# lbcb-sci/raven

Hardware: AMD Instinct MI355X
Metric: read Gbase/s through overlap+polish (higher is better)
Workload: dtype u32

## Files before the change

### raven_amd/csrc/engine.h

```cpp
#pragma once

#include <atomic>
#include <memory>
#include <mutex>
#include <string>
#include <vector>

#include "common.h"

namespace rvn {

constexpr int kSketchTile = 1024;
constexpr int kMaxWindow = 256;

inline u64 next_reads_serial() {
  static std::atomic<u64> counter{0};
  return ++counter;
}

struct ReadsDev {
  u32 n = 0;
  u64 total_bases = 0;
  u64 n_words = 0;
  DevBuf packed;
// ... 52 lines not shown
  DevBuf ovl_read_off;
  DevBuf filtered;
  bool has_anchors = false;
  DevBuf anchors;
  DevBuf anchor_off;
  DevBuf anchor_cnt;
};

struct StageTimes {
  enum { kSketch, kSort, kIndex, kFilter, kQuery, kMatch, kSegSort, kIntervals, kChain, kCompact, kMerge, kPile,
         kTruncate, kNum };
  double ms[kNum] = {};
  u64 launches[kNum] = {};
};

struct PileState;
struct PileRegion;
struct ResolveState;

struct EngineOptions {
  long long nw_budget_mb = 0;
  long long nw_group_walk = 0;
  long long nw_stripe_lanes = 0;
  long long index_direct_min_keys = 0;
  long long poa_rows_min_windows = -1;
  long long io_threads = 0;
  long long io_slab_mb = 0;
  long long io_ring = 0;
  long long io_zlib = 0;
  long long arena_mb = 0;
  long long arena_margin_mb = 0;
  long long no_arena = 0;
  long long release_always = 0;
  long long polish_join = 0;
  long long polish_sketch_cache_mb = -1;
};
const char* engine_option_names();
long long* engine_option(EngineOptions& o, const char* name);

struct Engine {
  EngineOptions opt;
  std::recursive_mutex mu;
  u32 k, w, bandwidth, chain, matches, gap;
  int device = 0;
  bool val64 = false;
  hipStream_t stream = nullptr;
// ... 164 lines not shown

struct NwJob;
struct NwWindowRec;
struct NwStats {
  u64 n_aligned = 0, n_retries = 0, n_unaligned = 0, n_batches = 0;
  u64 band_cells = 0, sum_distance = 0, store_bytes = 0;
  double ms = 0;
};
struct NwPathSlots {
  std::vector<std::unique_ptr<DevBuf>> blocks;
  std::vector<u64> slot_end;
};
void nw_breakpoints(Engine& e, const ReadsDev& T, const ReadsDev& R, std::vector<NwJob>& jobs, u32 w, NwWindowRec* d_recs,
                    u64 n_recs, NwStats& st, std::vector<u32>* distances = nullptr, NwPathSlots* path = nullptr);
struct NwPaths {
  u32 n = 0, n_not_aligned = 0;
  u64 n_runs = 0, n_ops = 0;
  std::vector<u32> distances;
  DevBuf run_off, runs, op_off;
  double device_ms = 0;
};
void nw_align_paths(Engine& e, const ReadsDev& T, const ReadsDev& Q, std::vector<NwJob>& jobs, NwPaths& out);
void nw_paths_expand(Engine& e, const NwPaths& p, u8* d_ops);
int nw_breakpoints_host(const u64* t_words, u32 t_len, const u64* r_words, u32 r_len, u32 t_begin, u32 n, u32 q_begin, u32 m,
                        int rc, u32 w, u32 k, int force_R, NwWindowRec* recs, u32* distance, u32* band);
void shard_split_minimizers(Engine& e, const u64* d_val, const u64* d_org, u64 n, u32 world, u64* d_val_out, u64* d_org_out,
                            u64* counts );
void shard_split_overlaps(Engine& e, const Overlap* d_ovl, u64 n, const u32* bounds , u32 world, u32 self,
                          Overlap* d_out, u64* counts );
u64 shard_count_flagged(Engine& e, const u64* d_org, u64 n);
void shard_adjacent_diff(Engine& e, const u64* d_seg, u64 n, u64* d_cnt);
void shard_regroup(Engine& e, u32 world, const u64* const* d_cnt, const u64* const* d_grp, const u64* const* d_pos,
                   const u64* n_src , u32 n_reads, u64* d_seg, u64* d_grp_out, u64* d_pos_out);
void shard_lhs_offsets(Engine& e, const Overlap* d_ovl, u64 n, u32 n_reads, u32* d_off);
struct PolishDirectOut {
  u8* out;
  const u64* off;
  u64* len;
};
void polish_map_best(Engine& e, ReadsDev& T, ReadsDev& R, u32 r_first, u32 r_last, double err_thr,
                     std::vector<Overlap>& best, std::vector<u32>& best_t, u64* n_overlaps);
void polish_round(Engine& e, ReadsDev& T, ReadsDev& R, const u8* h_quals, const u64* h_qual_off, double q_thr,
                  double err_thr, u32 w, bool trim, int m, int n, int g, std::vector<std::vector<u8>>& polished,
                  std::vector<double>& ratio, PolishStats& stats, u64 win_first = 0, u64 win_last = ~0ULL,
                  std::vector<u32>* win_count = nullptr, std::vector<u32>* win_polished = nullptr,
                  const PolishDirectOut* direct = nullptr);

struct Pass2State {
// ... 128 lines not shown
```

### raven_amd/csrc/engine.hip

```cpp
#include <chrono>
#include <memory>

#include "abi.h"
#include "poa.h"

using namespace rvn;

static_assert(sizeof(rvn_overlap) == sizeof(rvn::Overlap), "overlap layout");

namespace {

thread_local std::string g_err;

const char* kStageNames[StageTimes::kNum] = {"sketch", "sort", "index", "filter", "query_sketch", "match",
                                             "seg_sort", "intervals", "chain", "compact", "merge", "pile",
                                             "truncate"};

void swap_bufs(DevBuf& a, DevBuf& b) {
  std::swap(a.ptr, b.ptr);
  std::swap(a.cap, b.cap);
}

}

// ... 54 lines not shown
  }
  for (u32 i = first; i < last; ++i) e.c_index_bases += r.h_len[i];
  e.c_index_min += e.index_sketch.count;
  index_build(e, e.index_sketch, !(e.index.has_query_flags || e.index.all_query));
  e.c_index_keys += e.index.u;
  if (raw_handed_over) {
    if (e.raw_sketch.val.cap < e.index_sketch.val.cap) swap_bufs(e.raw_sketch.val, e.index_sketch.val);
    if (e.raw_sketch.org.cap < e.index_sketch.org.cap) swap_bufs(e.raw_sketch.org, e.index_sketch.org);
  }
}

void fetch_values(Engine& e, const DevBuf& val, u64 n, u64* values) {
  if (!values || n == 0) return;
  if (e.val64) {
    RVN_HIP(hipMemcpy(values, val.ptr, n * 8, hipMemcpyDeviceToHost));
  } else {
    std::vector<u32> tmp(n);
    RVN_HIP(hipMemcpy(tmp.data(), val.ptr, n * 4, hipMemcpyDeviceToHost));
    for (u64 i = 0; i < n; ++i) values[i] = tmp[i];
  }
}

const char* engine_option_names() {
  return "nw_budget_mb, nw_group_walk, nw_stripe_lanes, index_direct_min_keys, poa_rows_min_windows, io_threads, io_slab_mb, io_ring, io_zlib, arena_mb, arena_margin_mb, "
         "no_arena, release_always, polish_join, polish_sketch_cache_mb";
}
long long* engine_option(EngineOptions& o, const char* name) {
  const std::string n(name ? name : "");
  if (n == "nw_budget_mb") return &o.nw_budget_mb;
  if (n == "nw_group_walk") return &o.nw_group_walk;
  if (n == "nw_stripe_lanes") return &o.nw_stripe_lanes;
  if (n == "index_direct_min_keys") return &o.index_direct_min_keys;
  if (n == "poa_rows_min_windows") return &o.poa_rows_min_windows;
  if (n == "io_threads") return &o.io_threads;
  if (n == "io_slab_mb") return &o.io_slab_mb;
  if (n == "io_ring") return &o.io_ring;
  if (n == "io_zlib") return &o.io_zlib;
  if (n == "arena_mb") return &o.arena_mb;
  if (n == "arena_margin_mb") return &o.arena_margin_mb;
  if (n == "no_arena") return &o.no_arena;
  if (n == "release_always") return &o.release_always;
  if (n == "polish_join") return &o.polish_join;
  if (n == "polish_sketch_cache_mb") return &o.polish_sketch_cache_mb;
  return nullptr;
}

void engine_release_scratch(Engine& e) {
  if (e.stream) (void)rvn_stream_sync(e.stream);
  e.query_ready = false;
  DevBuf* bufs[] = {
      &e.index.s_val[0], &e.index.s_val[1], &e.index.s_org[0], &e.index.s_org[1], &e.index.u_val, &e.index.u_start,
      &e.index.table, &e.index.direct, &e.index_sketch.val, &e.index_sketch.org, &e.index_sketch.read_off, &e.query_sketch.val,
      &e.query_sketch.org, &e.query_sketch.read_off, &e.raw_sketch.val, &e.raw_sketch.org, &e.raw_sketch.read_off,
      &e.map_out.ovl, &e.map_out.ovl_read_off, &e.map_out.filtered, &e.map_out.anchors, &e.map_out.anchor_off,
// ... 223 lines not shown
```

### raven_amd/csrc/nwpath.hip

```cpp
#include <algorithm>
#include <mutex>
#include <chrono>
#include <cmath>
#include <cstdio>
#include <cstdlib>
#include <exception>
#include <type_traits>
#include <vector>

#include "engine.h"
#include "nwpath.h"
#include "nwsweep.h"
#include "nwtrace.h"
#include "wave.h"

namespace rvn {

namespace {

constexpr int kNwLaneStripCols = 16;
constexpr int kNwGroupLanes = 16;
constexpr u32 kNwGroupWalkMaxJobs = 8192;
constexpr u32 kSideSweepMaxWaves = 2048;
constexpr u32 kLevels = 8;
// ... 113 lines not shown
        }
        if ((t & 31) == 0) {
          const int qi = (t >> 5) - 1;
          if (st_ok && qi < n_q) {
            NwPm* p = ck_j + static_cast<u64>(qi - qc0) * row + static_cast<u64>(lig) * R;
#pragma unroll
            for (int r = 0; r < R; ++r) p[r] = NwPm{ln.Pv[r], ln.Mv[r]};
          }
        }
        ln.next_group(t);
        if (STRIPED && is_top) top.next_group(t);
      }
    }
    if (STRIPED && has && lig == lig_hand) hs_j[row * static_cast<u64>(gps)] = static_cast<u32>(sc_hand);
    const u32 res1 = group_max<G>(ln.result);
    if (has && lig == 0 && last) {
      const u32 res = res1 - 1u;
      result[ji] = res;
      status[ji] = (res1 != 0 && res <= k) ? 0u : 2u;
    }
  }
}

template <bool STRIP_LDS, int SC, class Out = NwWindowRec>
__global__ __launch_bounds__(64) void nw_trace_kernel(const NwJob* __restrict__ jobs, const u32* __restrict__ idx, u32 n_idx,
                                                      const u64* __restrict__ t_words, const u64* __restrict__ r_words,
                                                      const u32* __restrict__ hs, const NwPm* __restrict__ ck,
                                                      const u32* __restrict__ result, u32* __restrict__ status, u32 w,
                                                      Out* __restrict__ recs, u64* __restrict__ scratch) {
  __shared__ u64 s_pv[STRIP_LDS ? (SC + 1) * 64 : 1];
  __shared__ u64 s_mv[STRIP_LDS ? (SC + 1) * 64 : 1];
  __builtin_amdgcn_s_setprio(3);
  const u32 q = blockIdx.x * 64 + threadIdx.x;
  if (q >= n_idx) return;
  const u32 ji = idx[q];
  if (status[ji] != 0) return;
  const NwJob J = jobs[ji];
  const NwGeo geo = nw_geo_job(J);
  u64* g_pv = scratch + static_cast<u64>(blockIdx.x) * (2 * kNwStripCols * 64);
  const NwStripMem<64> mem{STRIP_LDS ? s_pv : g_pv, STRIP_LDS ? s_mv : g_pv + kNwStripCols * 64, static_cast<int>(threadIdx.x)};
  if constexpr (std::is_same<Out, u32>::value) {
    NwRunSink sink;
    sink.init(recs + J.bp_off, nw_slot_words(J.k));
    status[ji] = static_cast<u32>(nw_trace_job<64, SC, NwRunSink>(J, geo, t_words, r_words, hs + J.hs, ck + J.ckpt, mem, result[ji], w,
                                                                  nullptr, sink));
  } else {
// ... 36 lines not shown
    bad = G.walk_batch(geo, t == 0);
    __threadfence_block();
    __builtin_amdgcn_wave_barrier();
    if (bad) break;
  }
  const int rcode = bad ? 1 : G.wk.finish(t == 0);
  if (t == 0) status[ji] = static_cast<u32>(rcode);
}

template <int R, int G, bool STRIPED = false>
void launch_sweep(Engine& e, hipStream_t s, const NwJob* d_jobs, const u32* d_idx, u32 n_idx, const ReadsDev& T, const ReadsDev& Rd,
                  u32* d_hs, NwPm* d_ck, u32* d_result, u32* d_status, u32* d_next, int stripe = 0) {
  if (n_idx == 0) return;
  constexpr u32 NG = 64 / G;
  const u32 bundles = (n_idx + NG - 1) / NG;
  const u32 per_simd = static_cast<u32>(sweep_waves_per_simd<R>());
  const u32 waves = std::min<u32>(bundles, 256u * 4u * (per_simd > 4 ? per_simd - 2 : per_simd));
  RVN_HIP(hipMemsetAsync(d_next, 0, 4, s));
  RVN_KLAUNCH_ON(kKNwForward, s, (nw_sweep_kernel<R, G, STRIPED><<<(waves + 3) / 4, 256, 0, s>>>(
                               d_jobs, d_idx, n_idx, T.packed.as<u64>(), Rd.packed.as<u64>(), d_hs, d_ck, d_result,
                               d_status, d_next, stripe)));
}

u32 kcap_of(u32 n, u32 m, u32 R, u32 G) {
  const u32 d = n > m ? n - m : m - n;
  const u64 room = static_cast<u64>(G) * (64ULL * R + 1) - 64ULL * R;
  if (room < d) return 0;
  const u64 k = d + ((room - d) / 2) * 2 + 1;
  return static_cast<u32>(std::min<u64>(k, static_cast<u64>(n) + m));
}

u32 level_of(const NwJob& J) {
  if (J.S) return kStriped;
  for (u32 x = 0; x < kLevels; ++x)
    if (kRs[x] == J.R && kGs[x] == J.G) return x;
  return kLevels - 1;
}

}

void nw_breakpoints(Engine& e, const ReadsDev& T, const ReadsDev& Rd, std::vector<NwJob>& jobs, u32 w,
                    NwWindowRec* d_recs, u64 n_recs, NwStats& st, std::vector<u32>* distances, NwPathSlots* path) {
  st = NwStats();
  const u32 nj = static_cast<u32>(jobs.size());
  if (distances) distances->assign(nj, ~0u);
  if (path) path->slot_end.assign(nj, 0);
  hipStream_t s = e.stream;
  if (n_recs) RVN_HIP(hipMemsetAsync(d_recs, 0xFF, n_recs * sizeof(NwWindowRec), s));
  if (nj == 0) return;
  RVN_HIP(hipEventRecord(e.ev0, s));
  if (!e.nw_streams[0]) {
    int prio_least = 0, prio_greatest = 0;
    RVN_HIP(hipDeviceGetStreamPriorityRange(&prio_least, &prio_greatest));
    constexpr int kNwEv = static_cast<int>(sizeof(e.nw_ev) / sizeof(e.nw_ev[0]));
    hipStream_t made[8] = {nullptr, nullptr, nullptr, nullptr, nullptr, nullptr, nullptr, nullptr};
    hipEvent_t made_ev[kNwEv + 4] = {};
    try {
      for (int b = 0; b < 8; ++b) {
        if (b >= 3 && prio_greatest != prio_least)
          RVN_HIP(hipStreamCreateWithPriority(&made[b], hipStreamNonBlocking, prio_greatest));
        else
// ... 8 lines not shown
      throw;
    }
    for (int b = 0; b < 3; ++b) e.nw_side[b] = made[5 + b];
    for (int i = 0; i < 4; ++i) e.nw_side_ev[i] = made_ev[kNwEv + i];
    for (int i = 0; i < kNwEv; ++i) e.nw_ev[i] = made_ev[i];
    for (int b = 0; b < 5; ++b) e.nw_streams[b] = made[b];
  }
  struct WalkGuard {
    Engine& e;
    ~WalkGuard() {
      if (!std::uncaught_exceptions()) return;
      for (hipStream_t st2 : e.nw_streams)
        if (st2) (void)hipStreamSynchronize(st2);
      for (hipStream_t st2 : e.nw_side)
        if (st2) (void)hipStreamSynchronize(st2);
      (void)hipStreamSynchronize(e.stream);
    }
  } walk_guard{e};
  double rate = e.nw_rate > 0 ? e.nw_rate : 0.13;
  if (const char* ev = knob("RVN_NW_RATE")) rate = std::atof(ev);
  u64 budget = 0;
  const u32 stripe_lanes = e.opt.nw_stripe_lanes > 0 && e.opt.nw_stripe_lanes < 64 ? static_cast<u32>(e.opt.nw_stripe_lanes) : 64u;

  auto plan = [&](NwJob& J, u64 k) -> bool {
    const u32 d = J.n > J.m ? J.n - J.m : J.m - J.n;
    k = std::max<u64>(std::max<u64>(k, d), 16);
    k = std::min<u64>(k, static_cast<u64>(J.n) + J.m);
    J.S = 0;
    for (u32 lvl = 0; lvl < kLevels; ++lvl) {
      if (kGs[lvl] > stripe_lanes) continue;
      const u32 cap = kcap_of(J.n, J.m, kRs[lvl], kGs[lvl]);
      if (cap >= k) {
        J.R = kRs[lvl];
        J.G = kGs[lvl];
        J.k = static_cast<u32>(k);
        J.kcap = cap;
        return true;
      }
    }
    const u32 cap = kcap_of(J.n, J.m, 8, kNwMaxStripes * stripe_lanes);
    if (cap < k) return false;
    const NwGeo g = nw_geo_striped(J.n, J.m, static_cast<u32>(k), 8, stripe_lanes);
    if (g.hs_words() * 4 + g.ck_entries() * 16 > budget) return false;
    J.R = 8;
    J.G = 64;
    J.S = stripe_lanes;
    J.k = static_cast<u32>(k);
    J.kcap = cap;
    return true;
  };
  std::vector<u32> valid;
  for (u32 i = 0; i < nj; ++i) {
    const NwJob& J = jobs[i];
    if (J.n == 0 || J.m == 0 || J.n >= (1u << 30) || J.m >= (1u << 30)) ++st.n_unaligned;
    else valid.push_back(i);
  }

  {
    size_t free_b = 0, total_b = 0;
    RVN_HIP(hipMemGetInfo(&free_b, &total_b));
    const u64 held = e.nw_hs.cap + e.nw_ck.cap + e.nw_hs2.cap + e.nw_ck2.cap + e.nw_hs3.cap + e.nw_ck3.cap + e.nw_hs4.cap + e.nw_ck4.cap;
    budget = std::min<u64>((static_cast<u64>(free_b) + devpool::free_total()) / 4 + held, 64ULL << 30);
    if (e.opt.nw_budget_mb > 0) budget = static_cast<u64>(e.opt.nw_budget_mb) << 20;
    budget = std::max<u64>(budget, 64ULL << 20);
  }
  const bool trace_lds = !(knob("RVN_NW_TRACE_MEM") && std::atoi(knob("RVN_NW_TRACE_MEM")) == 1);
  const int group_walk = static_cast<int>(e.opt.nw_group_walk);
  const bool one_stream = knob("RVN_NW_ONE_STREAM") != nullptr;
  const bool dbg_sync = knob("RVN_NW_DEBUG") && std::atoi(knob("RVN_NW_DEBUG")) >= 2;
  std::vector<double> rates;
  rates.reserve(nj);
  std::vector<u32> h_result(nj), h_status(nj);
  constexpr u32 kHeadMax = 4096;
  NwJob* d_jobs = e.nw_jobs.get<NwJob>(static_cast<size_t>(nj) + 1 + 2 * kHeadMax);
  u32* d_res = e.nw_res.get<u32>(3 * static_cast<size_t>(nj) + 32 + 6 * kHeadMax);
  u32* d_status = d_res + nj + 1;
  u32* d_idx = d_status + nj + 1;
  u32* d_next = d_idx + nj + 1;
  struct PassDev {
    NwJob* jobs;
    u32 *idx, *res, *status;
    bool compact;
  };
  const PassDev dev_all{d_jobs, d_idx, d_res, d_status, false};
  const PassDev dev_head{d_jobs + nj + 1, d_next + 4 + 2 * kHeadMax, d_next + 4, d_next + 4 + kHeadMax, true};
  const PassDev dev_retry{dev_head.jobs + kHeadMax, dev_head.idx + 3 * kHeadMax, dev_head.res + 3 * kHeadMax,
                          dev_head.status + 3 * kHeadMax, true};
  u32* d_side_next = d_next + 4 + 6 * kHeadMax;
  bool side_pending[3] = {false, false, false};
  auto join_side = [&]() {
    for (int x = 0; x < 3; ++x) {
      if (side_pending[x]) RVN_HIP(hipStreamWaitEvent(s, e.nw_side_ev[x], 0));
      side_pending[x] = false;
    }
  };
  struct Obs {
    double len, d;
  };
  using clk = std::chrono::steady_clock;
  double h_plan = 0, h_order = 0, h_up = 0, h_res = 0;
  auto since = [](clk::time_point t) { return std::chrono::duration<double, std::milli>(clk::now() - t).count(); };
  std::vector<Obs> obs;
  struct Chunk {
    size_t c0, c1;
    u64 hs_w, ck_e;
    u32 coff[kClasses + 1];
  };
  DevBuf* hs_buf[4] = {&e.nw_hs, &e.nw_hs2, &e.nw_hs3, &e.nw_hs4};
  DevBuf* ck_buf[4] = {&e.nw_ck, &e.nw_ck2, &e.nw_ck3, &e.nw_ck4};
  bool set_used[4] = {false, false, false, false};
  struct Queued {
    std::vector<u32> order;
    PassDev dev;
    bool sweep_only;
    std::vector<u32> res, status;
  };
  std::vector<Queued> queued;
  std::vector<u8> early;
  enum Layout { kOwnFirst, kHeadOnly, kRotating };
  auto enqueue = [&](const std::vector<u32>& todo, bool sweep_only, Layout layout, const PassDev& dev, hipStream_t up,
                     std::vector<u32>* left) {
    if (todo.empty()) return;
    auto t_h = clk::now();
    std::vector<u32> order;
    {
      const size_t nt = todo.size();
      std::vector<u32> key(nt), tmp(nt), idx(nt);
      parallel_for(nt, 16384, [&](size_t x0, size_t x1) {
        for (size_t x = x0; x < x1; ++x) {
          const NwJob& J = jobs[todo[x]];
          const u32 mm = J.S ? std::min<u32>(nw_geo_job(J).n_stripes, (1u << 20) - 1) : std::min<u32>(J.m >> 3, (1u << 20) - 1);
          static_assert(kClasses <= 16, "4 bits of variant + 20 bits of length = the 24 key bits of the two passes");
          key[x] = 0xFFFFFFu - ((level_of(J) << 20) | mm);
          idx[x] = static_cast<u32>(x);
        }
      });
      for (int pass = 0; pass < 2; ++pass) {
        u32 cnt[4097] = {};
        const int sh = 12 * pass;
        for (size_t x = 0; x < nt; ++x) cnt[((key[idx[x]] >> sh) & 4095u) + 1]++;
        for (int c = 0; c < 4096; ++c) cnt[c + 1] += cnt[c];
        for (size_t x = 0; x < nt; ++x) tmp[cnt[(key[idx[x]] >> sh) & 4095u]++] = idx[x];
        idx.swap(tmp);
      }
      order.resize(nt);
      for (size_t x = 0; x < nt; ++x) order[x] = todo[idx[x]];
    }
    std::vector<Chunk> chunks;
    u64 slot_w = 0;
    struct Need {
      u64 hw, ce, cells;
      u32 level;
    };
    std::vector<Need> need(order.size());
    parallel_for(order.size(), 16384, [&](size_t x0, size_t x1) {
      for (size_t x = x0; x < x1; ++x) {
        const NwJob& J = jobs[order[x]];
        const NwGeo g = nw_geo_job(J);
        need[x] = Need{g.hs_words(), g.ck_entries(), static_cast<u64>(J.m) * (static_cast<u64>(g.lo) + g.hi + 1), level_of(J)};
      }
    });
    for (size_t c0 = 0; c0 < order.size();) {
      Chunk C{};
      C.c0 = c0;
      size_t c1 = c0;
      while (c1 < order.size()) {
        NwJob& J = jobs[order[c1]];
        const u64 hw = need[c1].hw, ce = need[c1].ce;
        const u64 share = (chunks.empty() && layout != kRotating) ? budget / 12 : budget / 3;
        if (c1 > c0 && (C.hs_w + hw) * 4 + (C.ck_e + ce) * 16 > share) break;
        J.hs = C.hs_w;
        J.ckpt = C.ck_e;
        if (path && !sweep_only) {
          J.bp_off = slot_w;
          slot_w += nw_slot_words(J.k);
        }
        C.hs_w += hw;
        C.ck_e += ce;
        st.band_cells += need[c1].cells;
        C.coff[need[c1].level + 1]++;
        ++c1;
      }
      u32 run_off = 0, cnt[kClasses];
      for (u32 x = 0; x < kClasses; ++x) cnt[x] = C.coff[x + 1];
      for (int x = static_cast<int>(kClasses) - 1; x >= 0; --x) {
        C.coff[x] = run_off;
        run_off += cnt[x];
      }
      C.coff[kClasses] = run_off;
      C.c1 = c1;
      st.store_bytes = std::max<u64>(st.store_bytes, C.hs_w * 4 + C.ck_e * 16);
      chunks.push_back(C);
      c0 = c1;
      if (layout == kHeadOnly) break;
    }
    if (layout == kHeadOnly && chunks[0].c1 < order.size()) {
      for (size_t x = chunks[0].c1; x < order.size(); ++x) left->push_back(order[x]);
      order.resize(chunks[0].c1);
    }
    auto set_of = [&](size_t ci) -> int {
      if (layout == kRotating) return static_cast<int>(ci % 3);
      return ci == 0 ? 3 : static_cast<int>((ci - 1) % 3);
    };
    for (int b = 0; b < 4; ++b) {
      u64 set_hs = 0, set_ck = 0;
// ... 11 lines not shown
    u64* d_strip = nullptr;
    if (!trace_lds) {
      size_t mc = 0;
      for (const Chunk& C : chunks) mc = std::max(mc, C.c1 - C.c0);
      d_strip = e.nw_strip.get<u64>(static_cast<size_t>((mc + 63) / 64) * 2 * kNwStripCols * 64 * 4 + 64);
    }
    u32* d_slots = nullptr;
    if (path && !sweep_only) {
      path->blocks.emplace_back(new DevBuf());
      d_slots = path->blocks.back()->get<u32>(slot_w + 16);
      for (u32 i : order) path->slot_end[i] = reinterpret_cast<u64>(d_slots + jobs[i].bp_off + nw_slot_words(jobs[i].k) - 1);
    }
    h_order += since(t_h);
    t_h = clk::now();
    if (dev.compact) {
      std::vector<NwJob> hj(order.size());
      std::vector<u32> iota(order.size());
      for (size_t x = 0; x < order.size(); ++x) {
        hj[x] = jobs[order[x]];
        iota[x] = static_cast<u32>(x);
      }
      RVN_HIP(hipMemcpyAsync(dev.jobs, hj.data(), hj.size() * sizeof(NwJob), hipMemcpyHostToDevice, up));
      RVN_HIP(hipMemcpyAsync(dev.idx, iota.data(), iota.size() * 4, hipMemcpyHostToDevice, up));
      RVN_HIP(rvn_stream_sync(up));
    } else {
      RVN_HIP(hipMemcpyAsync(dev.jobs, jobs.data(), static_cast<size_t>(nj) * sizeof(NwJob), hipMemcpyHostToDevice, up));
      RVN_HIP(hipMemcpyAsync(dev.idx, order.data(), order.size() * 4, hipMemcpyHostToDevice, up));
      RVN_HIP(rvn_stream_sync(up));
    }
    h_up += since(t_h);
    for (size_t ci = 0; ci < chunks.size(); ++ci) {
      const Chunk& C = chunks[ci];
      const int b = set_of(ci);
      u32* hs = hs_buf[b]->as<u32>();
      NwPm* ck = ck_buf[b]->as<NwPm>();
      const u32* idx_c = dev.idx + C.c0;
      const u32 cn = static_cast<u32>(C.c1 - C.c0);
      if (set_used[b]) RVN_HIP(hipStreamWaitEvent(s, e.nw_ev[b], 0));
      auto count_of = [&](u32 x) -> u32 {
        const u32 next_off = x == 0 ? cn : C.coff[x - 1];
        return next_off - C.coff[x];
      };
      hipStream_t ts = one_stream ? s : e.nw_streams[b];
      auto launch_walk_to = [&](auto* d_out, hipStream_t wst, const u32* idx_w, u32 n_w) {
        using Out = typename std::remove_pointer<decltype(d_out)>::type;
        if (group_walk == 2 || (group_walk != 1 && n_w <= kNwGroupWalkMaxJobs)) {
          constexpr u32 NG = 64 / kNwGroupLanes;
          RVN_KLAUNCH_ON(kKNwTraceback, wst, (nw_trace_group_kernel<kNwGroupLanes, Out><<<(n_w + NG - 1) / NG, 64, 0, wst>>>(
                                                 dev.jobs, idx_w, n_w, T.packed.as<u64>(), Rd.packed.as<u64>(), hs, ck, dev.res,
                                                 dev.status, w, d_out)));
// ... 3 lines not shown
                                                 dev.status, w, d_out, nullptr)));
        } else if (trace_lds) {
          RVN_KLAUNCH_ON(kKNwTraceback, wst, (nw_trace_kernel<true, kNwCkSteps, Out><<<(n_w + 63) / 64, 64, 0, wst>>>(
                                                 dev.jobs, idx_w, n_w, T.packed.as<u64>(), Rd.packed.as<u64>(), hs, ck, dev.res,
                                                 dev.status, w, d_out, nullptr)));
        } else {
          RVN_KLAUNCH_ON(kKNwTraceback, wst, (nw_trace_kernel<false, kNwCkSteps, Out><<<(n_w + 63) / 64, 64, 0, wst>>>(
                                                 dev.jobs, idx_w, n_w, T.packed.as<u64>(), Rd.packed.as<u64>(), hs, ck, dev.res,
                                                 dev.status, w, d_out,
                                                 d_strip + static_cast<size_t>(b) * ((e.nw_strip.cap / 32) & ~size_t(63)))));
        }
      };
      auto launch_walk = [&](hipStream_t wst, const u32* idx_w, u32 n_w) {
        if (path) launch_walk_to(d_slots, wst, idx_w, n_w);
        else launch_walk_to(d_recs, wst, idx_w, n_w);
      };
      bool side[kLevels] = {};
      bool side_used[3] = {false, false, false};
      {
        u32 n_levels = 0;
        for (u32 x = 0; x < kLevels; ++x) n_levels += count_of(x) ? 1u : 0u;
        if (n_levels >= 2 && !one_stream && !dbg_sync)
          for (u32 x = 0; x < kLevels; ++x) {
            const u32 bundles = (count_of(x) + 64 / kGs[x] - 1) / (64 / kGs[x]);
            side[x] = count_of(x) && bundles <= kSideSweepMaxWaves;
            if (side[x]) side_used[x % 3] = true;
          }
        if (side_used[0] || side_used[1] || side_used[2]) {
          RVN_HIP(hipEventRecord(e.nw_side_ev[3], s));
          for (int y = 0; y < 3; ++y)
            if (side_used[y]) RVN_HIP(hipStreamWaitEvent(e.nw_side[y], e.nw_side_ev[3], 0));
        }
      }
      if (const u32 n_str = count_of(kStriped)) {
        const u32* idx_s = idx_c + C.coff[kStriped];
        std::vector<u32> n_stripes(n_str);
        for (u32 x = 0; x < n_str; ++x) n_stripes[x] = static_cast<u32>(nw_geo_job(jobs[order[C.c0 + C.coff[kStriped] + x]]).n_stripes);
        for (u32 stp = 0;; ++stp) {
          u32 n_st = 0;
          while (n_st < n_str && n_stripes[n_st] > stp) ++n_st;
          if (n_st == 0) break;
          launch_sweep<8, 64, true>(e, s, dev.jobs, idx_s, n_st, T, Rd, hs, ck, dev.res, dev.status, d_next, static_cast<int>(stp));
          if (dbg_sync) {
            RVN_HIP(hipStreamSynchronize(s));
            std::fprintf(stderr, "[raven_hip] nw: stripe %u done, %u jobs\n", stp, n_st);
          }
        }
      }
#define RVN_SWEEP(x, R_, G_)                                                                                         \
  do {                                                                                                               \
    launch_sweep<R_, G_>(e, side[x] ? e.nw_side[(x) % 3] : s, dev.jobs, idx_c + C.coff[x], count_of(x), T, Rd, hs, ck, \
                         dev.res, dev.status, side[x] ? d_side_next + (x) : d_next);                                   \
    if (dbg_sync && count_of(x)) {                                                                                   \
      RVN_HIP(hipStreamSynchronize(s));                                                                              \
      std::fprintf(stderr, "[raven_hip] nw: sweep R=%d G=%d done, %u jobs\n", R_, G_, count_of(x));                   \
    }                                                                                                                \
  } while (0)
      RVN_SWEEP(7, 8, 64);
      RVN_SWEEP(6, 4, 64);
      RVN_SWEEP(5, 2, 64);
      RVN_SWEEP(4, 1, 64);
      RVN_SWEEP(3, 1, 32);
      RVN_SWEEP(2, 1, 16);
      RVN_SWEEP(1, 1, 8);
      RVN_SWEEP(0, 1, 4);
#undef RVN_SWEEP
      for (int y = 0; y < 3; ++y)
        if (side_used[y]) {
          RVN_HIP(hipEventRecord(e.nw_side_ev[y], e.nw_side[y]));
          side_pending[y] = true;
        }
      ++st.n_batches;
      if (sweep_only) continue;
      if (!one_stream) {
        RVN_HIP(hipEventRecord(e.nw_ev[4], s));
        RVN_HIP(hipStreamWaitEvent(ts, e.nw_ev[4], 0));
        for (int y = 0; y < 3; ++y)
          if (side_used[y]) RVN_HIP(hipStreamWaitEvent(ts, e.nw_side_ev[y], 0));
      }
      launch_walk(ts, idx_c, cn);
      if (!one_stream) {
        RVN_HIP(hipEventRecord(e.nw_ev[b], ts));
        set_used[b] = true;
      }
// ... 602 lines not shown
      continue;
    }
    J.R = kRs[lvl];
    J.G = kGs[lvl];
    J.k = static_cast<u32>(kk);
    J.kcap = cap;
    int rcode;
    switch (J.R) {
      case 1: rcode = emulate_job<1>(J, J.G, t_words, r_words, w, recs, distance, band, walk_gl); break;
      case 2: rcode = emulate_job<2>(J, J.G, t_words, r_words, w, recs, distance, band, walk_gl); break;
      case 4: rcode = emulate_job<4>(J, J.G, t_words, r_words, w, recs, distance, band, walk_gl); break;
      default: rcode = emulate_job<8>(J, J.G, t_words, r_words, w, recs, distance, band, walk_gl); break;
    }
    if (walk_gl && band) band[3] = static_cast<u32>(g_group_batches_store);
    if (rcode == -3 && !force_R) {
      kk = std::min<u64>(static_cast<u64>(cap) + 1, static_cast<u64>(n) + m);
      continue;
    }
    return rcode;
  }
  return -3;
}

#endif

}
```

### raven_amd/hip.py

```python
from __future__ import annotations

import ctypes as C
import os

import numpy as np

_HERE = os.path.dirname(os.path.abspath(__file__))
LIB_PATH = os.environ.get("RVN_LIB_PATH") or os.path.join(_HERE, "lib", "libraven_hip.so")
TEST_LIB_PATH = os.path.join(os.path.dirname(LIB_PATH), "libraven_hip_test.so")

OVERLAP_DTYPE = np.dtype([
    ("lhs_id", "<u4"), ("lhs_begin", "<u4"), ("lhs_end", "<u4"),
    ("rhs_id", "<u4"), ("rhs_begin", "<u4"), ("rhs_end", "<u4"),
    ("score", "<u4"), ("strand", "<u4")])

ED_PAIR_DTYPE = np.dtype([
    ("lhs_read", "<u4"), ("lhs_begin", "<u4"), ("lhs_len", "<u4"),
    ("rhs_read", "<u4"), ("rhs_begin", "<u4"), ("rhs_len", "<u4"),
    ("strand", "<u4"), ("reserved", "<u4")])

ALIGN_PAIR_DTYPE = np.dtype([
    ("query_read", "<u4"), ("query_begin", "<u4"), ("query_len", "<u4"),
    ("target_read", "<u4"), ("target_begin", "<u4"), ("target_len", "<u4"),
    ("strand", "<u4"), ("reserved", "<u4")])
# ... 1253 lines not shown


NW_REC_DTYPE = np.dtype([("first_t", "<u4"), ("first_q", "<u4"), ("last_t", "<u4"), ("last_q", "<u4"),
                         ("grid", "<u2", (8,))])


def test_nw_breakpoints(t_words, t_len, r_words, r_len, t_begin, n, q_begin, m, rc, w, k=64, force_r=0, group_lanes=0,
                       stripe_lanes=0, device=False):
    t_words = np.ascontiguousarray(t_words, dtype=np.uint64)
    r_words = np.ascontiguousarray(r_words, dtype=np.uint64)
    n_win = (t_begin + n - 1) // w - t_begin // w + 1
    recs = np.zeros(n_win, dtype=NW_REC_DTYPE)
    dist = np.zeros(1, dtype=np.uint32)
    band = np.zeros(5 if (stripe_lanes or device) else (4 if group_lanes else 3), dtype=np.uint32)
    flags = (1 if rc else 0) | (int(stripe_lanes) << 16) | (1 << 24 if device else int(group_lanes) << 8)
    rc_ = test_lib().rvn_test_nw_breakpoints(_p(t_words), t_len, _p(r_words), r_len, t_begin, n, q_begin, m, flags, w, k,
                                             force_r, _p(recs), _p(dist), _p(band))
    if rc_ < 0:
        raise ValueError("rvn_test_nw_breakpoints: %d" % rc_)
    if device:
        return recs, int(dist[0]), dict(k=int(band[0]), stripe_lanes=int(band[1]), R=int(band[2]), stripes=int(band[3]),
                                        stage_ms=band[4] / 1000.0), rc_
    return recs, int(dist[0]), tuple(int(x) for x in band), rc_
```

Measured before the change: 1.443.

## Pack multiple ring-1 NW sweep jobs into shared 64-lane waves

Adds a packed sweep kernel for R=1 Myers/NW jobs. Each job gets only as many lanes as its band needs, and a host-side bin-packer fills 64-lane wavefronts with several jobs, sorted by step count. Before, a narrow-band job occupied a whole wave. The path is on by default (only disabled when nw_sweep_pack==2) and adds host packing cost, a persistent atomic work queue, and more complex chunking. Idle lanes and mismatched step counts within a wave can still waste work.

```diff
diff --git a/raven_amd/csrc/engine.h b/raven_amd/csrc/engine.h
--- a/raven_amd/csrc/engine.h
+++ b/raven_amd/csrc/engine.h
@@ -98,6 +98,7 @@
   long long nw_budget_mb = 0;
   long long nw_group_walk = 0;
   long long nw_stripe_lanes = 0;
+  long long nw_sweep_pack = 0;
   long long index_direct_min_keys = 0;
   long long poa_rows_min_windows = -1;
   long long io_threads = 0;
@@ -308,8 +309,15 @@
 };
 void nw_align_paths(Engine& e, const ReadsDev& T, const ReadsDev& Q, std::vector<NwJob>& jobs, NwPaths& out);
 void nw_paths_expand(Engine& e, const NwPaths& p, u8* d_ops);
+struct NwPackPlan {
+  std::vector<u32> order, wrec;
+  u32 n_waves() const { return static_cast<u32>(wrec.size() / 3); }
+};
+void nw_pack_waves(const u32* lanes, const u32* steps, u32 n, NwPackPlan& plan);
 int nw_breakpoints_host(const u64* t_words, u32 t_len, const u64* r_words, u32 r_len, u32 t_begin, u32 n, u32 q_begin, u32 m,
                         int rc, u32 w, u32 k, int force_R, NwWindowRec* recs, u32* distance, u32* band);
+int nw_packed_wave_host(const u64* t_words, const u64* r_words, u32 r_len, u32 n_jobs, const u32* spans, u64 ring_starts, u32 w,
+                        NwWindowRec* recs, u32* distance, u32* status, u32* lanes);
 void shard_split_minimizers(Engine& e, const u64* d_val, const u64* d_org, u64 n, u32 world, u64* d_val_out, u64* d_org_out,
                             u64* counts );
 void shard_split_overlaps(Engine& e, const Overlap* d_ovl, u64 n, const u32* bounds , u32 world, u32 self,
diff --git a/raven_amd/csrc/engine.hip b/raven_amd/csrc/engine.hip
--- a/raven_amd/csrc/engine.hip
+++ b/raven_amd/csrc/engine.hip
@@ -100,7 +100,7 @@
 }
 
 const char* engine_option_names() {
-  return "nw_budget_mb, nw_group_walk, nw_stripe_lanes, index_direct_min_keys, poa_rows_min_windows, io_threads, io_slab_mb, io_ring, io_zlib, arena_mb, arena_margin_mb, "
+  return "nw_budget_mb, nw_group_walk, nw_stripe_lanes, nw_sweep_pack, index_direct_min_keys, poa_rows_min_windows, io_threads, io_slab_mb, io_ring, io_zlib, arena_mb, arena_margin_mb, "
          "no_arena, release_always, polish_join, polish_sketch_cache_mb";
 }
 long long* engine_option(EngineOptions& o, const char* name) {
@@ -108,6 +108,7 @@
   if (n == "nw_budget_mb") return &o.nw_budget_mb;
   if (n == "nw_group_walk") return &o.nw_group_walk;
   if (n == "nw_stripe_lanes") return &o.nw_stripe_lanes;
+  if (n == "nw_sweep_pack") return &o.nw_sweep_pack;
   if (n == "index_direct_min_keys") return &o.index_direct_min_keys;
   if (n == "poa_rows_min_windows") return &o.poa_rows_min_windows;
   if (n == "io_threads") return &o.io_threads;
diff --git a/raven_amd/csrc/nwpath.hip b/raven_amd/csrc/nwpath.hip
--- a/raven_amd/csrc/nwpath.hip
+++ b/raven_amd/csrc/nwpath.hip
@@ -159,6 +159,100 @@
   }
 }
 
+__host__ __device__ __forceinline__ void nw_packed_place(u64 starts, int lane, int& ring, int& gbase) {
+  const u64 upto = starts << (63 - lane);
+  ring = static_cast<int>(RVN_POPC64(upto)) - 1;
+#if defined(__HIP_DEVICE_COMPILE__)
+  gbase = lane - __clzll(static_cast<long long>(upto));
+#else
+  gbase = upto ? lane - __builtin_clzll(upto) : -1;
+#endif
+}
+
+__global__ __launch_bounds__(256) __attribute__((amdgpu_waves_per_eu(8)))
+void nw_sweep_packed_kernel(const NwJob* __restrict__ jobs, const u32* __restrict__ idx, const u32* __restrict__ wrec,
+                            u32 n_waves, const u64* __restrict__ t_words, const u64* __restrict__ r_words,
+                            u32* __restrict__ hs, NwPm* __restrict__ ck, u32* __restrict__ result, u32* __restrict__ status,
+                            u32* __restrict__ next) {
+  __shared__ u64 s_peq[4][4 * 64];
+  const int lane = lane_id();
+  u64* peq = s_peq[threadIdx.x >> 6];
+  for (;;) {
+    int lane_f = lane;
+    asm volatile("" : "+v"(lane_f));
+    u32 q0 = atomicAdd(next, lane_f == 0 ? 1u : 0u);
+    q0 = static_cast<u32>(__builtin_amdgcn_readfirstlane(static_cast<int>(q0)));
+    if (q0 >= n_waves) break;
+    u32 starts_lo = wrec[3 * static_cast<u64>(q0)], starts_hi = wrec[3 * static_cast<u64>(q0) + 1];
+    const u32 off = wrec[3 * static_cast<u64>(q0) + 2];
+    NwSweepLane<1, 64> ln;
+    const NwJob* J0 = jobs + idx[off];
+    u32* const hs0 = hs + J0->hs;
+    NwPm* const ck0 = ck + J0->ckpt;
+    u32 hs_o = 0, ck_o = 0;
+    int prev = lane;
+    {
+      int ring, gbase;
+      nw_packed_place(static_cast<u64>(starts_lo) | (static_cast<u64>(starts_hi) << 32), lane_f, ring, gbase);
+      const int lig = lane - gbase;
+      bool has = false;
+      if (ring >= 0) {
+        const NwJob J = jobs[idx[off + static_cast<u32>(ring)]];
+        const NwGeo geo = nw_geo(J.n, J.m, J.k, 1);
+        has = lig < geo.L;
+        if (has) {
+          ln.init(J, t_words, r_words, geo, lig, peq, lane);
+          hs_o = static_cast<u32>(J.hs - J0->hs) + static_cast<u32>(lig);
+          ck_o = static_cast<u32>(J.ckpt - J0->ckpt) + static_cast<u32>(lig);
+          prev = lig == 0 ? gbase + geo.L - 1 : lane - 1;
+        }
+      }
+      if (!has) ln.init_idle(peq, lane);
+    }
+    int n_steps_w = ln.g.m + ln.g.n_super;
+#pragma unroll
+    for (int o = 32; o > 0; o >>= 1) {
+      const int v = __shfl_xor(n_steps_w, o, 64);
+      n_steps_w = v > n_steps_w ? v : n_steps_w;
+    }
+    n_steps_w = __builtin_amdgcn_readfirstlane((n_steps_w + 15) & ~15);
+    __builtin_assume(n_steps_w >= 16);
+    for (int t = 1; t <= n_steps_w; ++t) {
+      const int x = __shfl(ln.xf, prev, 64);
+      if (__ballot(ln.has_event(t)) != 0) {
+        const int sp = __shfl(ln.sc, prev, 64);
+        if (ln.has_event(t)) ln.event(t, x, sp);
+      }
+      ln.step(t, x);
+      if ((t & 15) == 0) {
+        int n_steps = ln.g.m;
+        asm volatile("" : "+v"(n_steps));
+        n_steps += ln.g.n_super;
+        if (t < n_steps + kNwHsSteps) hs0[hs_o] = ln.acc[0];
+        hs_o += static_cast<u32>(ln.g.L);
+        if ((t & 31) == 0) {
+          if (t <= n_steps) ck0[ck_o] = NwPm{ln.Pv[0], ln.Mv[0]};
+          ck_o += static_cast<u32>(ln.g.L);
+        }
+        ln.next_group(t);
+      }
+    }
+    asm volatile("" : "+s"(starts_lo), "+s"(starts_hi));
+    asm volatile("" : "+v"(lane_f));
+    int ring, gbase;
+    nw_packed_place(static_cast<u64>(starts_lo) | (static_cast<u64>(starts_hi) << 32), lane_f, ring, gbase);
+    const int L = ln.g.L;
+    const u64 found = __ballot(ln.result != 0) & ((L >= 64 ? ~0ULL : (1ULL << L) - 1ULL) << (gbase & 63));
+    const u32 res1 = __shfl(ln.result, found ? static_cast<int>(__ffsll(static_cast<unsigned long long>(found))) - 1 : lane, 64);
+    if (ring >= 0 && lane == gbase && L > 0) {
+      const u32 ji = idx[off + static_cast<u32>(ring)];
+      const u32 res = (found ? res1 : 0u) - 1u;
+      result[ji] = res;
+      status[ji] = (found != 0 && res <= jobs[ji].k) ? 0u : 2u;
+    }
+  }
+}
+
 template <bool STRIP_LDS, int SC, class Out = NwWindowRec>
 __global__ __launch_bounds__(64) void nw_trace_kernel(const NwJob* __restrict__ jobs, const u32* __restrict__ idx, u32 n_idx,
                                                       const u64* __restrict__ t_words, const u64* __restrict__ r_words,
@@ -241,6 +335,16 @@
                                d_status, d_next, stripe)));
 }
 
+void launch_sweep_packed(Engine& e, hipStream_t s, const NwJob* d_jobs, const u32* d_idx, const u32* d_wrec, u32 n_waves,
+                         const ReadsDev& T, const ReadsDev& Rd, u32* d_hs, NwPm* d_ck, u32* d_result, u32* d_status, u32* d_next) {
+  if (n_waves == 0) return;
+  const u32 waves = std::min<u32>(n_waves, 256u * 4u * 6u);
+  RVN_HIP(hipMemsetAsync(d_next, 0, 4, s));
+  RVN_KLAUNCH_ON(kKNwForward, s, (nw_sweep_packed_kernel<<<(waves + 3) / 4, 256, 0, s>>>(
+                               d_jobs, d_idx, d_wrec, n_waves, T.packed.as<u64>(), Rd.packed.as<u64>(), d_hs, d_ck, d_result,
+                               d_status, d_next)));
+}
+
 u32 kcap_of(u32 n, u32 m, u32 R, u32 G) {
   const u32 d = n > m ? n - m : m - n;
   const u64 room = static_cast<u64>(G) * (64ULL * R + 1) - 64ULL * R;
@@ -249,13 +353,89 @@
   return static_cast<u32>(std::min<u64>(k, static_cast<u64>(n) + m));
 }
 
-u32 level_of(const NwJob& J) {
+constexpr u32 kPackedLevel = 4;
+u32 level_of(const NwJob& J, bool pack) {
   if (J.S) return kStriped;
+  if (pack && J.R == 1) return kPackedLevel;
   for (u32 x = 0; x < kLevels; ++x)
     if (kRs[x] == J.R && kGs[x] == J.G) return x;
   return kLevels - 1;
 }
 
+}
+
+void nw_pack_waves(const u32* lanes, const u32* steps, u32 n, NwPackPlan& plan) {
+  plan.order.clear();
+  plan.wrec.clear();
+  if (n == 0) return;
+  u32 max_steps = 0;
+  for (u32 i = 0; i < n; ++i) {
+    if (lanes[i] < 1 || lanes[i] > 64) throw HipError("[raven_hip] nw_pack_waves: a ring of 1 .. 64 lanes");
+    max_steps = std::max(max_steps, steps[i]);
+  }
+  std::vector<u64> srt(n), tmp(n);
+  for (u32 i = 0; i < n; ++i) srt[i] = (static_cast<u64>(max_steps - steps[i]) << 32) | i;
+  std::vector<u32> cnt(65537);
+  for (int sh = 0; sh < 32 && (max_steps >> sh) != 0; sh += 16) {
+    std::fill(cnt.begin(), cnt.end(), 0u);
+    for (u32 x = 0; x < n; ++x) cnt[((srt[x] >> (32 + sh)) & 65535u) + 1]++;
+    for (int c = 0; c < 65536; ++c) cnt[c + 1] += cnt[c];
+    for (u32 x = 0; x < n; ++x) tmp[cnt[(srt[x] >> (32 + sh)) & 65535u]++] = srt[x];
+    srt.swap(tmp);
+  }
+  u32 head[66] = {}, end[66] = {};
+  for (u32 i = 0; i < n; ++i) end[lanes[i]]++;
+  for (u32 l = 1, at = 0; l <= 64; ++l) {
+    head[l] = at;
+    at += end[l];
+    end[l] = at;
+  }
+  std::vector<u64>& bkt = tmp;
+  {
+    u32 fill[66];
+    for (u32 l = 0; l < 66; ++l) fill[l] = head[l];
+    for (u32 x = 0; x < n; ++x) {
+      const u32 job = static_cast<u32>(srt[x]);
+      bkt[fill[lanes[job]]++] = (static_cast<u64>(x) << 32) | job;
+    }
+  }
+  u32 top[65];
+  for (u32 l = 0; l <= 64; ++l) top[l] = l >= 1 && head[l] < end[l] ? static_cast<u32>(bkt[head[l]] >> 32) : n;
+  u32 min_l = 1;
+  plan.order.reserve(n);
+  plan.wrec.reserve(3 * static_cast<size_t>(n / 2 + 1));
+  std::vector<u8> placed(static_cast<size_t>(n) + 1, 0);
+  u32 lead = 0;
+  while (plan.order.size() < n) {
+    u32 free_l = 64;
+    u64 starts = 0;
+    const u32 off = static_cast<u32>(plan.order.size());
+    while (placed[lead]) ++lead;
+    while (min_l <= 64 && top[min_l] == n) ++min_l;
+    while (free_l >= min_l) {
+      u32 best = n, bl = 0;
+      if (free_l == 64) {
+        best = lead;
+        bl = lanes[static_cast<u32>(srt[lead])];
+      } else {
+        for (u32 l = min_l; l <= free_l; ++l) {
+          const bool lt = top[l] < best;
+          best = lt ? top[l] : best;
+          bl = lt ? l : bl;
+        }
+        if (best == n) break;
+      }
+      placed[best] = 1;
+      starts |= 1ULL << (64 - free_l);
+      plan.order.push_back(static_cast<u32>(bkt[head[bl]]));
+      ++head[bl];
+      top[bl] = head[bl] < end[bl] ? static_cast<u32>(bkt[head[bl]] >> 32) : n;
+      free_l -= bl;
+    }
+    plan.wrec.push_back(static_cast<u32>(starts));
+    plan.wrec.push_back(static_cast<u32>(starts >> 32));
+    plan.wrec.push_back(off);
+  }
 }
 
 void nw_breakpoints(Engine& e, const ReadsDev& T, const ReadsDev& Rd, std::vector<NwJob>& jobs, u32 w,
@@ -310,6 +490,8 @@
   u64 budget = 0;
   const u32 stripe_lanes = e.opt.nw_stripe_lanes > 0 && e.opt.nw_stripe_lanes < 64 ? static_cast<u32>(e.opt.nw_stripe_lanes) : 64u;
 
+  const bool pack = e.opt.nw_sweep_pack != 2;
+
   auto plan = [&](NwJob& J, u64 k) -> bool {
     const u32 d = J.n > J.m ? J.n - J.m : J.m - J.n;
     k = std::max<u64>(std::max<u64>(k, d), 16);
@@ -317,12 +499,17 @@
     J.S = 0;
     for (u32 lvl = 0; lvl < kLevels; ++lvl) {
       if (kGs[lvl] > stripe_lanes) continue;
+      if (pack && kRs[lvl] == 1 && static_cast<u64>(J.m) + (J.n + 63) / 64 > (1u << 30) - 16) continue;
       const u32 cap = kcap_of(J.n, J.m, kRs[lvl], kGs[lvl]);
       if (cap >= k) {
         J.R = kRs[lvl];
         J.G = kGs[lvl];
         J.k = static_cast<u32>(k);
         J.kcap = cap;
+        if (pack && J.R == 1) {
+          J.G = nw_ring_lanes(nw_band_lo(J.n, J.m, J.k), nw_band_hi(J.n, J.m, J.k), 1);
+          J.kcap = kcap_of(J.n, J.m, 1, J.G);
+        }
         return true;
       }
     }
@@ -361,7 +548,7 @@
   std::vector<u32> h_result(nj), h_status(nj);
   constexpr u32 kHeadMax = 4096;
   NwJob* d_jobs = e.nw_jobs.get<NwJob>(static_cast<size_t>(nj) + 1 + 2 * kHeadMax);
-  u32* d_res = e.nw_res.get<u32>(3 * static_cast<size_t>(nj) + 32 + 6 * kHeadMax);
+  u32* d_res = e.nw_res.get<u32>(6 * static_cast<size_t>(nj) + 40 + 12 * kHeadMax);
   u32* d_status = d_res + nj + 1;
   u32* d_idx = d_status + nj + 1;
   u32* d_next = d_idx + nj + 1;
@@ -369,12 +556,15 @@
     NwJob* jobs;
     u32 *idx, *res, *status;
     bool compact;
+    u32* wrec;
   };
-  const PassDev dev_all{d_jobs, d_idx, d_res, d_status, false};
-  const PassDev dev_head{d_jobs + nj + 1, d_next + 4 + 2 * kHeadMax, d_next + 4, d_next + 4 + kHeadMax, true};
+  u32* d_side_next = d_next + 4 + 6 * kHeadMax;
+  u32* d_wrec = d_side_next + 8;
+  const PassDev dev_all{d_jobs, d_idx, d_res, d_status, false, d_wrec};
+  const PassDev dev_head{d_jobs + nj + 1, d_next + 4 + 2 * kHeadMax, d_next + 4, d_next + 4 + kHeadMax, true,
+                         d_wrec + 3 * (static_cast<size_t>(nj) + 1)};
   const PassDev dev_retry{dev_head.jobs + kHeadMax, dev_head.idx + 3 * kHeadMax, dev_head.res + 3 * kHeadMax,
-                          dev_head.status + 3 * kHeadMax, true};
-  u32* d_side_next = d_next + 4 + 6 * kHeadMax;
+                          dev_head.status + 3 * kHeadMax, true, dev_head.wrec + 3 * kHeadMax};
   bool side_pending[3] = {false, false, false};
   auto join_side = [&]() {
     for (int x = 0; x < 3; ++x) {
@@ -391,6 +581,7 @@
   std::vector<Obs> obs;
   struct Chunk {
     size_t c0, c1;
+    u32 w0, w1;
     u64 hs_w, ck_e;
     u32 coff[kClasses + 1];
   };
@@ -411,15 +602,15 @@
     if (todo.empty()) return;
     auto t_h = clk::now();
     std::vector<u32> order;
-    {
-      const size_t nt = todo.size();
+    auto by_variant = [&](const std::vector<u32>& in) {
+      const size_t nt = in.size();
       std::vector<u32> key(nt), tmp(nt), idx(nt);
       parallel_for(nt, 16384, [&](size_t x0, size_t x1) {
         for (size_t x = x0; x < x1; ++x) {
-          const NwJob& J = jobs[todo[x]];
+          const NwJob& J = jobs[in[x]];
           const u32 mm = J.S ? std::min<u32>(nw_geo_job(J).n_stripes, (1u << 20) - 1) : std::min<u32>(J.m >> 3, (1u << 20) - 1);
           static_assert(kClasses <= 16, "4 bits of variant + 20 bits of length = the 24 key bits of the two passes");
-          key[x] = 0xFFFFFFu - ((level_of(J) << 20) | mm);
+          key[x] = 0xFFFFFFu - ((level_of(J, pack) << 20) | mm);
           idx[x] = static_cast<u32>(x);
         }
       });
@@ -431,8 +622,30 @@
         for (size_t x = 0; x < nt; ++x) tmp[cnt[(key[idx[x]] >> sh) & 4095u]++] = idx[x];
         idx.swap(tmp);
       }
-      order.resize(nt);
-      for (size_t x = 0; x < nt; ++x) order[x] = todo[idx[x]];
+      for (size_t x = 0; x < nt; ++x) order.push_back(in[idx[x]]);
+    };
+    NwPackPlan waves;
+    size_t n_wide = todo.size();
+    if (!pack) {
+      order.reserve(todo.size());
+      by_variant(todo);
+    } else {
+      std::vector<u32> wide, ring1;
+      for (u32 i : todo) (jobs[i].R == 1 && !jobs[i].S ? ring1 : wide).push_back(i);
+      n_wide = wide.size();
+      order.reserve(todo.size());
+      by_variant(wide);
+      std::vector<u32> lanes(ring1.size()), steps(ring1.size());
+      parallel_for(ring1.size(), 16384, [&](size_t x0, size_t x1) {
+        for (size_t x = x0; x < x1; ++x) {
+          const NwJob& J = jobs[ring1[x]];
+          lanes[x] = J.G;
+          steps[x] = static_cast<u32>(nw_geo(J.n, J.m, J.k, 1).n_steps);
+        }
+      });
+      nw_pack_waves(lanes.data(), steps.data(), static_cast<u32>(ring1.size()), waves);
+      for (u32 x : waves.order) order.push_back(ring1[x]);
+      for (size_t wv = 0; wv < waves.n_waves(); ++wv) waves.wrec[3 * wv + 2] += static_cast<u32>(n_wide);
     }
     std::vector<Chunk> chunks;
     u64 slot_w = 0;
@@ -445,30 +658,40 @@
       for (size_t x = x0; x < x1; ++x) {
         const NwJob& J = jobs[order[x]];
         const NwGeo g = nw_geo_job(J);
-        need[x] = Need{g.hs_words(), g.ck_entries(), static_cast<u64>(J.m) * (static_cast<u64>(g.lo) + g.hi + 1), level_of(J)};
+        need[x] = Need{g.hs_words(), g.ck_entries(), static_cast<u64>(J.m) * (static_cast<u64>(g.lo) + g.hi + 1), level_of(J, pack)};
       }
     });
+    u32 wv = 0;
     for (size_t c0 = 0; c0 < order.size();) {
       Chunk C{};
       C.c0 = c0;
+      C.w0 = wv;
       size_t c1 = c0;
       while (c1 < order.size()) {
-        NwJob& J = jobs[order[c1]];
-        const u64 hw = need[c1].hw, ce = need[c1].ce;
+        const size_t u1 = c1 < n_wide ? c1 + 1 : (wv + 1 < waves.n_waves() ? waves.wrec[3 * (static_cast<size_t>(wv) + 1) + 2] : order.size());
+        u64 hw = 0, ce = 0;
+        for (size_t x = c1; x < u1; ++x) {
+          hw += need[x].hw;
+          ce += need[x].ce;
+        }
         const u64 share = (chunks.empty() && layout != kRotating) ? budget / 12 : budget / 3;
         if (c1 > c0 && (C.hs_w + hw) * 4 + (C.ck_e + ce) * 16 > share) break;
-        J.hs = C.hs_w;
-        J.ckpt = C.ck_e;
-        if (path && !sweep_only) {
-          J.bp_off = slot_w;
-          slot_w += nw_slot_words(J.k);
-        }
-        C.hs_w += hw;
-        C.ck_e += ce;
-        st.band_cells += need[c1].cells;
-        C.coff[need[c1].level + 1]++;
-        ++c1;
-      }
+        for (; c1 < u1; ++c1) {
+          NwJob& J = jobs[order[c1]];
+          J.hs = C.hs_w;
+          J.ckpt = C.ck_e;
+          if (path && !sweep_only) {
+            J.bp_off = slot_w;
+            slot_w += nw_slot_words(J.k);
+          }
+          C.hs_w += need[c1].hw;
+          C.ck_e += need[c1].ce;
+          st.band_cells += need[c1].cells;
+          C.coff[need[c1].level + 1]++;
+        }
+        if (c1 > n_wide) ++wv;
+      }
+      C.w1 = wv;
       u32 run_off = 0, cnt[kClasses];
       for (u32 x = 0; x < kClasses; ++x) cnt[x] = C.coff[x + 1];
       for (int x = static_cast<int>(kClasses) - 1; x >= 0; --x) {
@@ -526,10 +749,12 @@
       }
       RVN_HIP(hipMemcpyAsync(dev.jobs, hj.data(), hj.size() * sizeof(NwJob), hipMemcpyHostToDevice, up));
       RVN_HIP(hipMemcpyAsync(dev.idx, iota.data(), iota.size() * 4, hipMemcpyHostToDevice, up));
+      if (wv) RVN_HIP(hipMemcpyAsync(dev.wrec, waves.wrec.data(), static_cast<size_t>(wv) * 12, hipMemcpyHostToDevice, up));
       RVN_HIP(rvn_stream_sync(up));
     } else {
       RVN_HIP(hipMemcpyAsync(dev.jobs, jobs.data(), static_cast<size_t>(nj) * sizeof(NwJob), hipMemcpyHostToDevice, up));
       RVN_HIP(hipMemcpyAsync(dev.idx, order.data(), order.size() * 4, hipMemcpyHostToDevice, up));
+      if (wv) RVN_HIP(hipMemcpyAsync(dev.wrec, waves.wrec.data(), static_cast<size_t>(wv) * 12, hipMemcpyHostToDevice, up));
       RVN_HIP(rvn_stream_sync(up));
     }
     h_up += since(t_h);
@@ -579,7 +804,7 @@
         for (u32 x = 0; x < kLevels; ++x) n_levels += count_of(x) ? 1u : 0u;
         if (n_levels >= 2 && !one_stream && !dbg_sync)
           for (u32 x = 0; x < kLevels; ++x) {
-            const u32 bundles = (count_of(x) + 64 / kGs[x] - 1) / (64 / kGs[x]);
+            const u32 bundles = pack && x == kPackedLevel ? C.w1 - C.w0 : (count_of(x) + 64 / kGs[x] - 1) / (64 / kGs[x]);
             side[x] = count_of(x) && bundles <= kSideSweepMaxWaves;
             if (side[x]) side_used[x % 3] = true;
           }
@@ -616,7 +841,17 @@
       RVN_SWEEP(7, 8, 64);
       RVN_SWEEP(6, 4, 64);
       RVN_SWEEP(5, 2, 64);
-      RVN_SWEEP(4, 1, 64);
+      if (pack) {
+        const bool sd = side[kPackedLevel];
+        launch_sweep_packed(e, sd ? e.nw_side[kPackedLevel % 3] : s, dev.jobs, dev.idx, dev.wrec + 3 * static_cast<size_t>(C.w0), C.w1 - C.w0, T,
+                            Rd, hs, ck, dev.res, dev.status, sd ? d_side_next + kPackedLevel : d_next);
+        if (dbg_sync && C.w1 > C.w0) {
+          RVN_HIP(hipStreamSynchronize(s));
+          std::fprintf(stderr, "[raven_hip] nw: packed sweep done, %u jobs in %u waves\n", count_of(kPackedLevel), C.w1 - C.w0);
+        }
+      } else {
+        RVN_SWEEP(4, 1, 64);
+      }
       RVN_SWEEP(3, 1, 32);
       RVN_SWEEP(2, 1, 16);
       RVN_SWEEP(1, 1, 8);
@@ -1265,6 +1500,96 @@
   return -3;
 }
 
+int nw_packed_wave_host(const u64* t_words, const u64* r_words, u32 r_len, u32 n_jobs, const u32* spans, u64 ring_starts, u32 w,
+                        NwWindowRec* recs, u32* distance, u32* status, u32* lanes_out) {
+  if (n_jobs == 0 || n_jobs > 64 || !(ring_starts & 1ULL) || static_cast<u32>(__builtin_popcountll(ring_starts)) != n_jobs) return -2;
+  std::vector<NwJob> jobs(n_jobs);
+  std::vector<NwGeo> geo(n_jobs);
+  std::vector<std::vector<u32>> hs(n_jobs);
+  std::vector<std::vector<NwPm>> ck(n_jobs);
+  u64 n_recs = 0;
+  for (u32 x = 0; x < n_jobs; ++x) {
+    const u32* sp = spans + 6 * static_cast<size_t>(x);
+    NwJob& J = jobs[x];
+    J = NwJob{};
+    J.t_begin = sp[0];
+    J.n = sp[1];
+    J.q_begin = sp[2];
+    J.m = sp[3];
+    J.r_len = r_len;
+    J.rc = sp[4] ? 1 : 0;
+    if (J.n == 0 || J.m == 0) return -1;
+    const u32 d = J.n > J.m ? J.n - J.m : J.m - J.n;
+    J.k = static_cast<u32>(std::min<u64>(std::max<u64>(std::max<u64>(sp[5], d), 1), static_cast<u64>(J.n) + J.m));
+    J.R = 1;
+    J.n_windows = (J.t_begin + J.n - 1) / w - J.t_begin / w + 1;
+    J.bp_off = n_recs;
+    n_recs += J.n_windows;
+    geo[x] = nw_geo(J.n, J.m, J.k, 1);
+    J.G = static_cast<u32>(geo[x].L);
+    lanes_out[x] = J.G;
+    hs[x].assign(geo[x].hs_words() + 4 * 64 * 8 + 16, 0xA5A5A5A5u);
+    ck[x].assign(geo[x].ck_entries() + 16, NwPm{0x1234567887654321ULL, 0x0FEDCBA99ABCDEF0ULL});
+  }
+  for (u64 x = 0; x < n_recs; ++x) {
+    recs[x].first_t = recs[x].first_q = recs[x].last_t = recs[x].last_q = 0xFFFFFFFFu;
+    for (int g = 0; g < 8; ++g) recs[x].grid[g] = 0xFFFFu;
+  }
+  std::vector<u64> peq(4 * 64);
+  std::vector<NwSweepLane<1, 64>> ln(64);
+  int ring[64], gbase[64], lig[64], prev[64], xp[64], sp_[64];
+  bool has[64];
+  int n_steps_w = 0;
+  for (int l = 0; l < 64; ++l) {
+    nw_packed_place(ring_starts, l, ring[l], gbase[l]);
+    lig[l] = l - gbase[l];
+    const int L = geo[ring[l]].L;
+    if (lig[l] == 0 && l + L > 64) return -3;
+    if (lig[l] == 0 && l + L < 64 && (ring_starts & (((1ULL << L) - 1ULL) << l)) != (1ULL << l)) return -3;
+    has[l] = lig[l] < L;
+    if (has[l]) ln[l].init(jobs[ring[l]], t_words, r_words, geo[ring[l]], lig[l], peq.data(), l);
+    else ln[l].init_idle(peq.data(), l);
+    if (has[l]) n_steps_w = std::max(n_steps_w, geo[ring[l]].n_steps);
+    prev[l] = lig[l] == 0 ? gbase[l] + L - 1 : l - 1;
+  }
+  n_steps_w = (n_steps_w + 15) & ~15;
+  for (int t = 1; t <= n_steps_w; ++t) {
+    for (int l = 0; l < 64; ++l) {
+      xp[l] = ln[prev[l]].xf;
+      sp_[l] = ln[prev[l]].sc;
+    }
+    for (int l = 0; l < 64; ++l)
+      if (ln[l].has_event(t)) ln[l].event(t, xp[l], sp_[l]);
+    for (int l = 0; l < 64; ++l) ln[l].step(t, xp[l]);
+    if ((t & 15) == 0) {
+      const int gi = (t >> 4) - 1, qi = (t >> 5) - 1;
+      for (int l = 0; l < 64; ++l) {
+        if (!has[l]) continue;
+        const NwGeo& g = geo[ring[l]];
+        const int n_g = (g.n_steps + kNwHsSteps - 1) / kNwHsSteps, n_q = g.n_steps / kNwCkSteps;
+        const u64 row = static_cast<u64>(g.L);
+        if (gi < n_g) hs[ring[l]][static_cast<u64>(gi) * row + static_cast<u64>(lig[l])] = ln[l].acc[0];
+        if ((t & 31) == 0 && qi < n_q) ck[ring[l]][static_cast<u64>(qi) * row + static_cast<u64>(lig[l])] = NwPm{ln[l].Pv[0], ln[l].Mv[0]};
+      }
+      for (int l = 0; l < 64; ++l) ln[l].next_group(t);
+    }
+  }
+  u64 ballot = 0;
+  for (int l = 0; l < 64; ++l)
+    if (ln[l].result != 0) ballot |= 1ULL << l;
+  for (int l = 0; l < 64; ++l) {
+    if (!has[l] || lig[l] != 0) continue;
+    const u32 x = static_cast<u32>(ring[l]);
+    const int L = geo[x].L;
+    const u64 found = ballot & ((L >= 64 ? ~0ULL : (1ULL << L) - 1ULL) << gbase[l]);
+    const u32 res = (found ? ln[__builtin_ctzll(found)].result : 0u) - 1u;
+    distance[x] = res;
+    status[x] = (found != 0 && res <= jobs[x].k) ? 0u : 2u;
+    if (status[x] == 0) status[x] = static_cast<u32>(walk_host(jobs[x], geo[x], t_words, r_words, hs[x], ck[x], res, w, recs, nullptr, 0));
+  }
+  return 0;
+}
+
 #endif
 
 }
diff --git a/raven_amd/hip.py b/raven_amd/hip.py
--- a/raven_amd/hip.py
+++ b/raven_amd/hip.py
@@ -1299,3 +1299,43 @@
         return recs, int(dist[0]), dict(k=int(band[0]), stripe_lanes=int(band[1]), R=int(band[2]), stripes=int(band[3]),
                                         stage_ms=band[4] / 1000.0), rc_
     return recs, int(dist[0]), tuple(int(x) for x in band), rc_
+
+
+def test_nw_packed_wave(t_words, t_len, r_words, r_len, spans, ring_starts, w):
+    t_words = np.ascontiguousarray(t_words, dtype=np.uint64)
+    r_words = np.ascontiguousarray(r_words, dtype=np.uint64)
+    spans = np.ascontiguousarray(spans, dtype=np.uint32).reshape(-1, 6)
+    nj = spans.shape[0]
+    n_win = [(int(s[0]) + int(s[1]) - 1) // w - int(s[0]) // w + 1 for s in spans]
+    recs = np.zeros(sum(n_win), dtype=NW_REC_DTYPE)
+    dist = np.zeros(nj, dtype=np.uint32)
+    mask = 0
+    for b in ring_starts:
+        mask |= 1 << int(b)
+    band = np.concatenate([spans.ravel(), np.array([mask & 0xFFFFFFFF, mask >> 32], dtype=np.uint32)])
+    rc_ = test_lib().rvn_test_nw_breakpoints(_p(t_words), t_len, _p(r_words), r_len, 0, nj, 0, 0, 1 << 25, w, 0, 0, _p(recs),
+                                             _p(dist), _p(band))
+    if rc_ != 0:
+        raise ValueError("rvn_test_nw_breakpoints (packed wave): %d" % rc_)
+    cuts = np.cumsum([0] + n_win)
+    return [(recs[cuts[x]:cuts[x + 1]], int(dist[x]), int(band[x]), int(band[nj + x])) for x in range(nj)]
+
+
+def test_nw_pack_waves(n, m, k):
+    n, m, k = (np.ascontiguousarray(a, dtype=np.uint32) for a in (n, m, k))
+    cnt = n.shape[0]
+    assert m.shape[0] == cnt and k.shape[0] == cnt
+    band = np.concatenate([n, m, k, np.zeros(1, dtype=np.uint32)])
+    out = np.zeros(6 * cnt + 3, dtype=np.uint32)
+    nw = np.zeros(1, dtype=np.uint32)
+    rc_ = test_lib().rvn_test_nw_breakpoints(None, 0, None, 0, 0, cnt, 0, 0, 1 << 26, 0, 0, 0, _p(out), _p(nw), _p(band))
+    if rc_ != 0:
+        raise ValueError("rvn_test_nw_breakpoints (pack waves): %d" % rc_)
+    lanes, steps, order, wrec = out[:cnt].copy(), out[cnt:2 * cnt].copy(), out[2 * cnt:3 * cnt], out[3 * cnt:]
+    waves = []
+    for x in range(int(nw[0])):
+        mask = int(wrec[3 * x]) | (int(wrec[3 * x + 1]) << 32)
+        off = int(wrec[3 * x + 2])
+        starts = [b for b in range(64) if (mask >> b) & 1]
+        waves.append([(int(order[off + r]), b) for r, b in enumerate(starts)])
+    return lanes, steps, waves
```

After: 1.432. No clear change (-0.8%).
